# xswang/xflow

Measured on NVIDIA H100. Metric: training examples/sec, higher is better.
Workload: dtype f32

## Files before the change

### xflow_b200/csrc/step_lazy.cu

```cuda
#include <cuda_runtime.h>
#include <stdint.h>
#include <stdlib.h>

#include "kernels.h"
#include "table.cuh"

#define XF_NO_SLOT 0xFFFFFFFFu
#define XF_LAZY_CACHED 2

template <bool ADMIT, bool STAMP>
__device__ __forceinline__ bool xf_lazy_look(const XfTableView& t, uint64_t key, uint64_t& s, uint32_t& i, uint64_t& q0,
                                             uint64_t& q1, uint64_t& q2, uint64_t& q3, uint32_t& slot, bool& created,
                                             const XfAdmitView& adm, bool& rejected, const XfStampView& sv) {
  if (q0 == key) { slot = (uint32_t)s; return true; }
  if (q0 == XF_EMPTY_KEY) {
    if (ADMIT && !xf_admit(adm, key)) {
      rejected = adm.mode != XF_ADM_NEVER;
      return true;
    }
    const unsigned long long old =
        atomicCAS(reinterpret_cast<unsigned long long*>(xf_row(t, s)), (unsigned long long)XF_EMPTY_KEY, (unsigned long long)key);
    if (old == XF_EMPTY_KEY) {
      if (STAMP) sv.stamp[s] = sv.now;
      created = true;
      q0 = key; q1 = q2 = q3 = 0ull;
      slot = (uint32_t)s;
      return true;
    }
    if (old == key) {
      q0 = key;
      slot = (uint32_t)s;
      return true;
    }
  }
  if (++i == XF_MAX_PROBE) { *t.error = 1; return true; }
  s = xf_probe_slot(t, key, i);
  return false;
}

template <bool ADMIT, bool STAMP, bool WEIGHT>
__global__ void __launch_bounds__(256, 2)
xf_k_step_lr_lazy(XfTableView t, const uint32_t* __restrict__ row_ptr, const uint64_t* __restrict__ keys,
                  const uint8_t* __restrict__ labels, int B, int mode, uint32_t seq, uint64_t* rows_by_seq, int fix_shift,
                  float* __restrict__ loss_out, float* __restrict__ pctr_out, float* __restrict__ abs_loss_sum,
                  unsigned long long* __restrict__ unique_total, XfAdmitView adm, XfStampView sv, XfWeightView wv) {
  __shared__ float s_abs[8];
  __shared__ unsigned int s_open;
  if (WEIGHT) fix_shift = xf_fix_shift(*wv.W);
  __shared__ uint64_t s_q2[2 * XF_LAZY_CACHED][256], s_q3[2 * XF_LAZY_CACHED][256], s_q2n[2 * XF_LAZY_CACHED][256];
  if (threadIdx.x == 0) s_open = 0;
  if (blockIdx.x == 0 && threadIdx.x == 0 && mode == 0)
    rows_by_seq[seq] = (uint64_t)(uint32_t)B | ((uint64_t)fix_shift << 32);
  __syncthreads();
  float abs_acc = 0.f;
  unsigned int open_acc = 0;
  const int lane = threadIdx.x & 31;
  const int warps_per_block = blockDim.x >> 5;
  const int gwarp = blockIdx.x * warps_per_block + (threadIdx.x >> 5);
  const int nwarps = gridDim.x * warps_per_block;

  for (int row = gwarp; row < B; row += nwarps) {
    if (WEIGHT && __ldg(wv.e + row) == 0.f) {
      if (lane == 0 && loss_out) loss_out[row] = 0.f;
      continue;
    }
    const uint32_t beg = __ldg(row_ptr + row);
    const uint32_t end = __ldg(row_ptr + row + 1);
    const int chunks = (int)((end - beg + 63u) >> 6);
    const uint8_t label = mode == 0 ? labels[row] : 0;
    uint64_t k1_0 = 0ull, k1_1 = 0ull;
    if (beg + 64u + (uint32_t)lane < end) k1_0 = __ldcs(keys + beg + 64u + lane);
    if (beg + 96u + (uint32_t)lane < end) k1_1 = __ldcs(keys + beg + 96u + lane);
    float wsum = 0.f;
    uint32_t lead_s[2 * XF_LAZY_CACHED];
    uint32_t cnt_c[XF_LAZY_CACHED];
#pragma unroll
    for (int c = 0; c < XF_LAZY_CACHED; ++c) {
      lead_s[2 * c] = lead_s[2 * c + 1] = XF_NO_SLOT;
      cnt_c[c] = 0;
    }

    for (int ch = 0; ch < chunks; ++ch) {
      const uint32_t j0 = beg + (uint32_t)ch * 64u + (uint32_t)lane;
      const uint32_t j1 = j0 + 32u;
      const bool v0 = j0 < end, v1 = j1 < end;
      uint64_t k0 = k1_0, k1 = k1_1;
      if (ch != 1) {
        k0 = v0 ? __ldcs(keys + j0) : 0ull;
        k1 = v1 ? __ldcs(keys + j1) : 0ull;
      }
      uint64_t p0 = xf_home_slot(t, k0), p1 = xf_home_slot(t, k1);
      uint64_t a0, a1, a2, a3, b0, b1, b2, b3;
      xf_ld32_pair(v0 ? xf_row(t, p0) : nullptr, a0, a1, a2, a3);
      xf_ld32_pair(v1 ? xf_row(t, p1) : nullptr, b0, b1, b2, b3);
      uint32_t s0 = XF_NO_SLOT, s1 = XF_NO_SLOT, i0 = 0, i1 = 0;
      bool u0 = v0, u1 = v1, r0 = false, r1 = false;
      for (;;) {
        bool c0 = false, c1 = false;
        if (u0) u0 = !xf_lazy_look<ADMIT, STAMP>(t, k0, p0, i0, a0, a1, a2, a3, s0, c0, adm, r0, sv);
        if (u1) u1 = !xf_lazy_look<ADMIT, STAMP>(t, k1, p1, i1, b0, b1, b2, b3, s1, c1, adm, r1, sv);
        const unsigned created = __popc(__ballot_sync(0xffffffffu, c0)) + __popc(__ballot_sync(0xffffffffu, c1));
        if (created && lane == 0) {
          atomicAdd(t.size, (unsigned long long)created);
          if (ADMIT) atomicAdd(adm.admitted, (unsigned long long)created);
        }
        if (!__any_sync(0xffffffffu, u0 || u1)) break;
        uint64_t x0, x1, x2, x3;
        xf_ld32_pair(u0 ? xf_row(t, p0) : nullptr, x0, x1, x2, x3);
        if (u0) { a0 = x0; a1 = x1; a2 = x2; a3 = x3; }
        xf_ld32_pair(u1 ? xf_row(t, p1) : nullptr, x0, x1, x2, x3);
        if (u1) { b0 = x0; b1 = x1; b2 = x2; b3 = x3; }
      }
      if (ADMIT) xf_admit_append(adm, r0, k0, r1, k1);
      uint64_t a2n = a2, b2n = b2;
      float w0 = 0.f, w1 = 0.f;
      if (s0 != XF_NO_SLOT) w0 = xf_lazy_fold(t, a1, a2, a3, mode == 1 ? 0xFFFFFFFFu : seq, a2n);
      if (s1 != XF_NO_SLOT) w1 = xf_lazy_fold(t, b1, b2, b3, mode == 1 ? 0xFFFFFFFFu : seq, b2n);
      wsum += w0;
      wsum += w1;
      if (mode == 1) continue;
      const unsigned grp0 = __match_any_sync(0xffffffffu, (s0 != XF_NO_SLOT) ? s0 : (0xFFFFFF00u | (uint32_t)lane));
      const unsigned grp1 = __match_any_sync(0xffffffffu, (s1 != XF_NO_SLOT) ? s1 : (0xFFFFFF00u | (uint32_t)lane));
      const bool L0 = s0 != XF_NO_SLOT && lane == __ffs(grp0) - 1, L1 = s1 != XF_NO_SLOT && lane == __ffs(grp1) - 1;
      if (ch >= XF_LAZY_CACHED) {
        if (L0 && xf_lazy_deposit(t, xf_row(t, s0), a2, a3, a2n, seq, 0ll)) {
          ++open_acc;
          if (STAMP) sv.stamp[s0] = sv.now;
        }
        if (L1 && xf_lazy_deposit(t, xf_row(t, s1), b2, b3, b2n, seq, 0ll)) {
          ++open_acc;
          if (STAMP) sv.stamp[s1] = sv.now;
        }
      }
#pragma unroll
      for (int c = 0; c < XF_LAZY_CACHED; ++c)
        if (ch == c) {
          lead_s[2 * c] = L0 ? s0 : XF_NO_SLOT;
          lead_s[2 * c + 1] = L1 ? s1 : XF_NO_SLOT;
          cnt_c[c] = (L0 ? (uint32_t)__popc(grp0) : 0u) | ((L1 ? (uint32_t)__popc(grp1) : 0u) << 8);
        }
      if (ch < XF_LAZY_CACHED) {
        if (L0) { s_q2[2 * ch][threadIdx.x] = a2; s_q3[2 * ch][threadIdx.x] = a3; s_q2n[2 * ch][threadIdx.x] = a2n; }
        if (L1) { s_q2[2 * ch + 1][threadIdx.x] = b2; s_q3[2 * ch + 1][threadIdx.x] = b3; s_q2n[2 * ch + 1][threadIdx.x] = b2n; }
      }
    }

    const float wx = xf_warp_sum(wsum);
    const float pctr = xf_sigmoid(wx);
    if (mode == 1) {
      if (lane == 0 && pctr_out) pctr_out[row] = pctr;
      continue;
    }
    float loss = __fsub_rn(pctr, (float)label);
    if (lane == 0 && loss_out) loss_out[row] = loss;
    if (WEIGHT) loss = __fmul_rn(__ldg(wv.e + row), loss);
    abs_acc += fabsf(loss);
    const long long lf = xf_fix_of(loss, fix_shift);
    uint64_t o2[2 * XF_LAZY_CACHED], o3[2 * XF_LAZY_CACHED];
    bool issued[2 * XF_LAZY_CACHED];
#pragma unroll
    for (int g = 0; g < 2 * XF_LAZY_CACHED; ++g) {
      const int x = threadIdx.x;
      issued[g] = lead_s[g] != XF_NO_SLOT &&
                  xf_lazy_deposit_issue(xf_row(t, lead_s[g]), s_q2[g][x], s_q3[g][x], s_q2n[g][x], seq,
                                        lf * (long long)((cnt_c[g >> 1] >> (8 * (g & 1))) & 0xFFu), o2[g], o3[g]);
    }
#pragma unroll
    for (int g = 0; g < 2 * XF_LAZY_CACHED; ++g) {
      const int x = threadIdx.x;
      bool stale = false;
      if (issued[g] && xf_lazy_deposit_resolve(xf_row(t, lead_s[g]), true, s_q2[g][x], s_q3[g][x], o2[g], o3[g], seq,
                                               lf * (long long)((cnt_c[g >> 1] >> (8 * (g & 1))) & 0xFFu), &stale)) {
        ++open_acc;
        if (STAMP) sv.stamp[lead_s[g]] = sv.now;
      }
      if (stale) *t.error = 2;
    }
    for (int ch = XF_LAZY_CACHED; ch < chunks; ++ch) {
      const uint32_t j0 = beg + (uint32_t)ch * 64u + (uint32_t)lane;
      const uint32_t j1 = j0 + 32u;
      XfHead h;
      if (j0 < end) { const int64_t r = xf_probe<false>(t, __ldg(keys + j0), &h); if (r >= 0) xf_lazy_add(xf_row(t, (uint64_t)r), lf); }
      if (j1 < end) { const int64_t r = xf_probe<false>(t, __ldg(keys + j1), &h); if (r >= 0) xf_lazy_add(xf_row(t, (uint64_t)r), lf); }
    }
  }
  if (mode == 0) {
    if (lane == 0) s_abs[threadIdx.x >> 5] = abs_acc;
    if (open_acc) atomicAdd(&s_open, open_acc);
    __syncthreads();
    if (threadIdx.x == 0) {
      if (abs_loss_sum != nullptr) {
        float tot = 0.f;
        for (int w = 0; w < (int)(blockDim.x >> 5); ++w) tot += s_abs[w];
        atomicAdd(abs_loss_sum, tot);
      }
      if (unique_total != nullptr && s_open) atomicAdd(unique_total, (unsigned long long)s_open);
    }
  }
}

template <bool A, bool S, bool W>
static int xf_lazy_ctas_per_sm() {
  static const int n = [] {
    int v = 0;
    if (cudaOccupancyMaxActiveBlocksPerMultiprocessor(&v, xf_k_step_lr_lazy<A, S, W>, 256, 0) != cudaSuccess || v < 1) {
      cudaGetLastError();
      v = 1;
    }
    return v;
  }();
  return n;
}

void xf_launch_step_lr_lazy(const XfTableView& t, const uint32_t* row_ptr, const uint64_t* keys,
                            const uint8_t* labels, int B, uint64_t nnz, int mode, uint32_t seq, uint64_t* rows_by_seq,
                            float* loss_out, float* pctr_out, float* abs_loss_sum, unsigned long long* unique_total,
                            const XfAdmitView* adm, const XfStampView& sv, const XfWeightView& wv, cudaStream_t st) {
  if (B <= 0) return;
  const int fs = xf_fix_shift(nnz);
  const XfAdmitView a = adm ? *adm : XfAdmitView{};
#define XF_LAZY_ARGS t, row_ptr, keys, labels, B, mode, seq, rows_by_seq, fs, loss_out, pctr_out, abs_loss_sum, unique_total, a, sv, wv
#define XF_LAZY_LAUNCH(A, S, W)                                                                                      \
  xf_k_step_lr_lazy<A, S, W><<<xf_grid_for((uint64_t)B * 32, 256, xf_lazy_ctas_per_sm<A, S, W>()), 256, 0, st>>>( \
      XF_LAZY_ARGS)
#define XF_LAZY_LAUNCH_W(A, S)            \
  do {                                    \
    if (wv.e) XF_LAZY_LAUNCH(A, S, true); \
    else XF_LAZY_LAUNCH(A, S, false);     \
  } while (0)
  const bool stamp = sv.stamp != nullptr;
  if (adm && stamp) XF_LAZY_LAUNCH_W(true, true);
  else if (adm) XF_LAZY_LAUNCH_W(true, false);
  else if (stamp) XF_LAZY_LAUNCH_W(false, true);
  else XF_LAZY_LAUNCH_W(false, false);
#undef XF_LAZY_LAUNCH_W
#undef XF_LAZY_LAUNCH
#undef XF_LAZY_ARGS
}
```

### xflow_b200/csrc/table.cuh

```cuda
#pragma once
#include <cuda_runtime.h>
#include <stdint.h>

#define XF_EMPTY_KEY 0xFFFFFFFFFFFFFFFFull
#define XF_FLAG_V_READY 1u
#define XF_NEG_ZERO_BITS 0x80000000u
#define XF_NEG_ZERO_BITS64 0x8000000000000000ull
#define XF_MAX_PROBE 8192

enum { XF_OPT_FTRL = 0, XF_OPT_SGD = 1 };
enum { XF_INIT_DEFAULT = 0, XF_INIT_COUNTER = 1, XF_INIT_ZERO = 3 };

struct XfTableView {
  uint8_t* base;
  uint64_t mask;
  uint32_t log2cap;
  uint32_t bshift;
  uint32_t stride;
  int K;
  int opt;
  int v_init;
  float v_const;
  uint64_t seed;
  float alpha, beta, lambda1, lambda2, learning_rate;
  unsigned long long* size;
  int* error;
  int lazy;
  const uint64_t* rows_by_seq;
  int canon;
};
#define XF_ADM_POISSON 1
#define XF_ADM_BLOOM 2
#define XF_ADM_NEVER 3
#define XF_ADM_MAX_HASHES 8
struct XfAdmitView {
  int mode;
  uint32_t p24;
  uint64_t batch_mix;
  uint32_t threshold, log2_cells, hashes;
  uint64_t seed;
  const uint8_t* cells;
  unsigned long long* rej_n;
  uint64_t* rej_keys;
  unsigned long long* admitted;
};
struct XfKeep {
  uint32_t cutoff;
  int bounded;
  uint32_t s_star;
  uint64_t k_star;
};
struct XfStampView {
  uint32_t* stamp;
  uint32_t now;
};
struct XfWeightView {
  const float* e;
  const unsigned long long* W;
};
__host__ __device__ __forceinline__ bool xf_keeps(const XfKeep& k, uint32_t stamp, uint64_t key) {
  return stamp >= k.cutoff && (!k.bounded || stamp > k.s_star || (stamp == k.s_star && key <= k.k_star));
}
#define XF_TAG_LOCKED 0xFFFFFFFFu
#define XF_FIX_MAX_SHIFT 27
#define XF_TAG_MASK 0xFFFFull

__host__ __device__ inline int xf_fix_shift(uint64_t nnz) {
  int bits = 0;
  while (bits < 64 && (nnz >> bits) != 0ull) ++bits;
  const int s = 47 - bits;
  return s > XF_FIX_MAX_SHIFT ? XF_FIX_MAX_SHIFT : (s < 0 ? 0 : s);
}

__host__ __device__ inline uint32_t xf_acc_off(int K) { return (32u + 4u * (uint32_t)K + 15u) & ~15u; }
__host__ __device__ inline uint32_t xf_ca_off(int K, int opt) {
  return xf_acc_off(K) + 16u + ((opt == XF_OPT_FTRL) ? 8u * (uint32_t)K : 0u);
}
__host__ __device__ inline uint32_t xf_row_stride(int K, int opt, int canon = 0) {
  if (K <= 0) return 32u;
  uint32_t bytes = xf_ca_off(K, opt) + (canon ? 4u * (uint32_t)K : 0u);
  return (bytes + 31u) & ~31u;
}

#ifdef __CUDACC__

__device__ __forceinline__ uint64_t xf_probe_slot(const XfTableView& t, uint64_t key, uint32_t i) {
  const uint64_t m = key * 0x9E3779B97F4A7C15ull;
  const uint32_t bs = t.bshift;
  const uint64_t hb = m >> (64 - (t.log2cap - bs));
  const uint32_t b1 = (1u << bs) - 1u;
  const uint32_t j0 = (uint32_t)(m >> 9) & b1;
  const uint32_t k = i >> bs;
  const uint32_t j = (k == 0) ? ((j0 + i) & b1) : (i & b1);
  return (((hb + k) << bs) | j) & t.mask;
}
__device__ __forceinline__ uint64_t xf_home_slot(const XfTableView& t, uint64_t key) { return xf_probe_slot(t, key, 0); }

__host__ __device__ __forceinline__ uint64_t xf_splitmix64(uint64_t x) {
  x += 0x9E3779B97F4A7C15ull;
  x = (x ^ (x >> 30)) * 0xBF58476D1CE4E5B9ull;
  x = (x ^ (x >> 27)) * 0x94D049BB133111EBull;
  return x ^ (x >> 31);
}
__host__ __device__ __forceinline__ uint64_t xf_admit_cell(uint64_t key, uint64_t seed, uint32_t j, uint32_t log2_cells) {
  return xf_splitmix64(key ^ xf_splitmix64(seed + (uint64_t)(j + 1) * 0x9E3779B97F4A7C15ull)) >> (64 - log2_cells);
}
__device__ __forceinline__ bool xf_admit(const XfAdmitView& a, uint64_t key) {
  if (a.mode == XF_ADM_POISSON) return (uint32_t)(xf_splitmix64(key ^ a.batch_mix) >> 40) < a.p24;
  if (a.mode != XF_ADM_BLOOM) return false;
  uint32_t m = 255u;
  for (uint32_t j = 0; j < a.hashes; ++j) m = min(m, (uint32_t)__ldcg(a.cells + xf_admit_cell(key, a.seed, j, a.log2_cells)));
  return m >= a.threshold;
}
__device__ __forceinline__ void xf_admit_append(const XfAdmitView& a, bool r0, uint64_t k0, bool r1, uint64_t k1) {
  const unsigned m0 = __ballot_sync(0xffffffffu, r0), m1 = __ballot_sync(0xffffffffu, r1);
  if ((m0 | m1) == 0u) return;
  const unsigned lane = threadIdx.x & 31u;
  unsigned long long base = 0ull;
  if (lane == 0u) base = atomicAdd(a.rej_n, (unsigned long long)(__popc(m0) + __popc(m1)));
  base = __shfl_sync(0xffffffffu, base, 0);
  if (a.rej_keys) {
    const unsigned lt = (1u << lane) - 1u;
    if (r0) a.rej_keys[base + __popc(m0 & lt)] = k0;
    if (r1) a.rej_keys[base + __popc(m0) + __popc(m1 & lt)] = k1;
  }
}

__device__ __forceinline__ float xf_counter_normal(uint64_t key, uint32_t k, uint64_t seed) {
  uint64_t base = xf_splitmix64(key ^ xf_splitmix64(seed + 0x632BE59BD9B4E019ull * (uint64_t)(k + 1)));
  uint32_t sum = 0;
#pragma unroll
  for (int r = 0; r < 3; ++r) {
    uint64_t x = xf_splitmix64(base + (uint64_t)r);
    sum += (uint32_t)(x & 0xFFFF) + (uint32_t)((x >> 16) & 0xFFFF) + (uint32_t)((x >> 32) & 0xFFFF) +
           (uint32_t)((x >> 48) & 0xFFFF);
  }
  float u = __fmul_rn((float)((int32_t)sum - 6 * 65535), 1.0f / 65536.0f);
  return __fmul_rn(u, 1e-2f);
}
__device__ __forceinline__ float xf_v_init(const XfTableView& t, uint64_t key, uint32_t k) {
  if (t.v_init == XF_INIT_COUNTER) return xf_counter_normal(key, k, t.seed);
  if (t.v_init == XF_INIT_ZERO) return 0.0f;
  return t.v_const;
}

__device__ __forceinline__ uint8_t* xf_row(const XfTableView& t, uint64_t slot) {
  return t.base + slot * (uint64_t)t.stride;
}
__device__ __forceinline__ double* xf_row_g(uint8_t* row) { return reinterpret_cast<double*>(row + 8); }
#define XF_OFF_STATE 16
#define XF_OFF_FLAGS 28
__device__ __forceinline__ float* xf_row_v(uint8_t* row) { return reinterpret_cast<float*>(row + 32); }
__device__ __forceinline__ double* xf_row_acc(uint8_t* row, int K) { return reinterpret_cast<double*>(row + xf_acc_off(K)); }
__device__ __forceinline__ float* xf_row_nv(uint8_t* row, int K) { return reinterpret_cast<float*>(row + xf_acc_off(K) + 16); }
__device__ __forceinline__ float* xf_row_zv(uint8_t* row, int K) { return xf_row_nv(row, K) + K; }
__device__ __forceinline__ float* xf_row_ca(const XfTableView& t, uint8_t* row) { return reinterpret_cast<float*>(row + xf_ca_off(t.K, t.opt)); }

struct XfHead {
  uint64_t key;
  uint32_t flags;
  float w, n, z;
  double g;
};

__device__ __forceinline__ void xf_ld32_cg(const void* p, uint64_t& q0, uint64_t& q1, uint64_t& q2, uint64_t& q3) {
  asm volatile("ld.global.cg.v2.u64 {%0,%1}, [%4];\n\tld.global.cg.v2.u64 {%2,%3}, [%4+16];"
               : "=l"(q0), "=l"(q1), "=l"(q2), "=l"(q3) : "l"(p));
}
__device__ __forceinline__ void xf_ld32_ca(const void* p, uint64_t& q0, uint64_t& q1, uint64_t& q2, uint64_t& q3) {
  asm volatile("ld.global.ca.v2.u64 {%0,%1}, [%4];\n\tld.global.ca.v2.u64 {%2,%3}, [%4+16];"
               : "=l"(q0), "=l"(q1), "=l"(q2), "=l"(q3) : "l"(p));
}
__device__ __forceinline__ void xf_ld32_pair(const uint8_t* mine, uint64_t& q0, uint64_t& q1, uint64_t& q2, uint64_t& q3) {
  const uint32_t odd = threadIdx.x & 1u;
  const uint8_t* other = (const uint8_t*)__shfl_xor_sync(0xffffffffu, (unsigned long long)mine, 1);
  const uint8_t* r0 = odd ? other : mine;
  const uint8_t* r1 = odd ? mine : other;
  uint64_t x0 = 0, x1 = 0, y0 = 0, y1 = 0;
  asm volatile("{\n .reg .pred p0, p1;\n setp.ne.u64 p0, %4, 0;\n setp.ne.u64 p1, %5, 0;\n"
               " @p0 ld.global.cg.v2.u64 {%0,%1}, [%6];\n @p1 ld.global.cg.v2.u64 {%2,%3}, [%7];\n}"
               : "+l"(x0), "+l"(x1), "+l"(y0), "+l"(y1)
               : "l"(r0), "l"(r1), "l"(r0 + 16 * odd), "l"(r1 + 16 * odd));
  const uint64_t m0 = odd ? y0 : x0, m1 = odd ? y1 : x1;
  const uint64_t t0 = __shfl_xor_sync(0xffffffffu, odd ? x0 : y0, 1);
  const uint64_t t1 = __shfl_xor_sync(0xffffffffu, odd ? x1 : y1, 1);
  q0 = odd ? t0 : m0; q1 = odd ? t1 : m1;
  q2 = odd ? m0 : t0; q3 = odd ? m1 : t1;
}
__device__ __forceinline__ void xf_st32(void* p, uint64_t q0, uint64_t q1, uint64_t q2, uint64_t q3) {
  asm volatile("st.global.v2.u64 [%0], {%1,%2};\n\tst.global.v2.u64 [%0+16], {%3,%4};" ::"l"(p), "l"(q0), "l"(q1),
               "l"(q2), "l"(q3)
               : "memory");
}

__device__ __forceinline__ XfHead xf_load_head(const uint8_t* row) {
  uint64_t q0, q1, q2, q3;
  xf_ld32_cg(row, q0, q1, q2, q3);
  XfHead h;
  h.key = q0;
  h.g = __longlong_as_double((long long)q1);
  h.w = __uint_as_float((uint32_t)q2);
  h.n = __uint_as_float((uint32_t)(q2 >> 32));
  h.z = __uint_as_float((uint32_t)q3);
  h.flags = (uint32_t)(q3 >> 32);
  return h;
}

__device__ __forceinline__ XfHead xf_load_head_l1(const uint8_t* row) {
  uint64_t q0, q1, q2, q3;
  xf_ld32_ca(row, q0, q1, q2, q3);
  XfHead h;
  h.key = q0;
  h.g = __longlong_as_double((long long)q1);
  h.w = __uint_as_float((uint32_t)q2);
  h.n = __uint_as_float((uint32_t)(q2 >> 32));
  h.z = __uint_as_float((uint32_t)q3);
  h.flags = (uint32_t)(q3 >> 32);
  return h;
}

__device__ __forceinline__ void xf_ld8_l1(const float* p, float (&o)[8]) {
  uint64_t q0, q1, q2, q3;
  xf_ld32_ca(p, q0, q1, q2, q3);
  o[0] = __uint_as_float((uint32_t)q0); o[1] = __uint_as_float((uint32_t)(q0 >> 32));
  o[2] = __uint_as_float((uint32_t)q1); o[3] = __uint_as_float((uint32_t)(q1 >> 32));
  o[4] = __uint_as_float((uint32_t)q2); o[5] = __uint_as_float((uint32_t)(q2 >> 32));
  o[6] = __uint_as_float((uint32_t)q3); o[7] = __uint_as_float((uint32_t)(q3 >> 32));
}

template <int VEC>
__device__ __forceinline__ void xf_ldv_step(const float* p, float (&o)[VEC]) {
  if (VEC == 4) { float4 t = __ldca(reinterpret_cast<const float4*>(p)); o[0] = t.x; o[1 % VEC] = t.y; o[2 % VEC] = t.z; o[3 % VEC] = t.w; }
  else if (VEC == 2) { float2 t = __ldca(reinterpret_cast<const float2*>(p)); o[0] = t.x; o[1 % VEC] = t.y; }
  else { o[0] = __ldca(p); }
}
template <int VEC>
__device__ __forceinline__ void xf_fm_token(const XfTableView& t, uint32_t slot, uint32_t flags, uint64_t key,
                                            float& st, float& qt) {
  const int K = t.K;
  st = 0.f;
  qt = 0.f;
  if ((flags & XF_FLAG_V_READY) && (K & 7) == 0) {
    const float* vp = reinterpret_cast<const float*>(xf_row(t, slot) + 32);
    for (int k = 0; k < K; k += 8) {
      float v[8];
      xf_ld8_l1(vp + k, v);
#pragma unroll
      for (int e = 0; e < 8; ++e) { st += v[e]; qt = __fadd_rn(qt, __fmul_rn(v[e], v[e])); }
    }
  } else if (flags & XF_FLAG_V_READY) {
    const float* vp = reinterpret_cast<const float*>(xf_row(t, slot) + 32);
    for (int k = 0; k < K; k += VEC) {
      float v[VEC];
      xf_ldv_step<VEC>(vp + k, v);
#pragma unroll
      for (int e = 0; e < VEC; ++e) { st += v[e]; qt = __fadd_rn(qt, __fmul_rn(v[e], v[e])); }
    }
  } else {
    for (int k = 0; k < K; ++k) {
      const float v = xf_v_init(t, key, (uint32_t)k);
      st += v;
      qt = __fadd_rn(qt, __fmul_rn(v, v));
    }
  }
}

__device__ __forceinline__ void xf_store_head(uint8_t* row, const XfHead& h) {
  const uint64_t q1 = (uint64_t)__double_as_longlong(h.g);
  const uint64_t q2 = (uint64_t)__float_as_uint(h.w) | ((uint64_t)__float_as_uint(h.n) << 32);
  const uint64_t q3 = (uint64_t)__float_as_uint(h.z) | ((uint64_t)h.flags << 32);
  xf_st32(row, h.key, q1, q2, q3);
}

template <bool INSERT, bool ADMIT = false, bool STAMP = false>
__device__ __forceinline__ int64_t xf_probe_from(const XfTableView& t, uint64_t key, uint64_t s, XfHead& h,
                                                 const XfAdmitView* adm = nullptr, bool* rejected = nullptr,
                                                 const XfStampView* sv = nullptr) {
  for (int probes = 0; probes < XF_MAX_PROBE; ++probes) {
    if (h.key == key) return (int64_t)s;
    if (h.key == XF_EMPTY_KEY) {
      if (!INSERT) return -1;
      if (ADMIT && !xf_admit(*adm, key)) {
        *rejected = adm->mode != XF_ADM_NEVER;
        return -1;
      }
      unsigned long long old =
          atomicCAS(reinterpret_cast<unsigned long long*>(xf_row(t, s)), (unsigned long long)XF_EMPTY_KEY,
                    (unsigned long long)key);
      if (old == XF_EMPTY_KEY) {
        unsigned m = __activemask();
        int leader = __ffs(m) - 1;
        if ((int)(threadIdx.x & 31) == leader) {
          atomicAdd(t.size, (unsigned long long)__popc(m));
          if (ADMIT) atomicAdd(adm->admitted, (unsigned long long)__popc(m));
        }
        if (STAMP && sv->stamp != nullptr) sv->stamp[s] = sv->now;
        h.key = key; h.flags = 0; h.w = 0.f; h.n = 0.f; h.z = 0.f;
        h.g = t.lazy ? 0.0 : -0.0;
        return (int64_t)s;
      }
      if (old == key) {
        h.key = key;
        return (int64_t)s;
      }
    }
    s = xf_probe_slot(t, key, (uint32_t)probes + 1u);
    h = xf_load_head(xf_row(t, s));
  }
  *t.error = 1;
  return -1;
}

template <bool INSERT, bool STAMP = false>
__device__ __forceinline__ int64_t xf_probe(const XfTableView& t, uint64_t key, XfHead* head,
                                            const XfStampView* sv = nullptr) {
  const uint64_t s = xf_home_slot(t, key);
  XfHead h = xf_load_head(xf_row(t, s));
  const int64_t r = xf_probe_from<INSERT, false, STAMP>(t, key, s, h, nullptr, nullptr, sv);
  *head = h;
  return r;
}


__device__ __forceinline__ float xf_sigmoid(float x) {
  if (x < -30.f) return (float)1e-6;
  if (x > 30.f) return 1.0f;
  const double ex = exp((double)x * 0.9999999998311266);
  return (float)(ex / (1.0 + ex));
}

__device__ __forceinline__ void xf_ftrl_coord(const XfTableView& t, float g, float& w, float& n, float& z) {
  float old_n = n;
  float nn = __fadd_rn(old_n, __fmul_rn(g, g));
  float sig = __fdiv_rn(__fsub_rn(__fsqrt_rn(nn), __fsqrt_rn(old_n)), t.alpha);
  z = __fadd_rn(z, __fsub_rn(g, __fmul_rn(sig, w)));
  n = nn;
  if (fabsf(z) <= t.lambda1) {
    w = 0.0f;
  } else {
    float tmpr = 0.0f;
    if (z > 0.0f) tmpr = __fsub_rn(z, t.lambda1);
    if (z < 0.0f) tmpr = __fadd_rn(z, t.lambda1);
    float tmpl = -__fadd_rn(__fdiv_rn(__fadd_rn(t.beta, __fsqrt_rn(n)), t.alpha), t.lambda2);
    w = __fdiv_rn(tmpr, tmpl);
  }
}

__device__ __forceinline__ void xf_sgd_coord(const XfTableView& t, float g, float& w) {
  w = __fsub_rn(w, __fmul_rn(t.learning_rate, g));
}

__device__ __forceinline__ void xf_opt_coord(const XfTableView& t, float g, float& w, float& n, float& z) {
  if (t.opt == XF_OPT_FTRL) xf_ftrl_coord(t, g, w, n, z);
  else xf_sgd_coord(t, g, w);
}

__device__ __forceinline__ float xf_div_rows_plain(float g, double rows) { return (float)((double)g / rows); }
__device__ __forceinline__ float xf_div_rows(float g, double rows) {
  const long long b = __double_as_longlong(rows);
  if ((b & 0x000FFFFFFFFFFFFFll) == 0ll && b > 0ll) {
    const double inv = __longlong_as_double((2046ll << 52) - b);
    return (float)((double)g * inv);
  }
  return (float)((double)g / rows);
}

__device__ __forceinline__ float xf_ftrl_w(const XfTableView& t, float z, float n) {
  if (fabsf(z) <= t.lambda1) return 0.0f;
  float tmpr = 0.0f;
  if (z > 0.0f) tmpr = __fsub_rn(z, t.lambda1);
  if (z < 0.0f) tmpr = __fadd_rn(z, t.lambda1);
  const float tmpl = -__fadd_rn(__fdiv_rn(__fadd_rn(t.beta, __fsqrt_rn(n)), t.alpha), t.lambda2);
  return __fdiv_rn(tmpr, tmpl);
}
__device__ __forceinline__ double xf_pow2(int e) { return __longlong_as_double((long long)(1023 + e) << 52); }
__device__ __forceinline__ long long xf_fix_of(float residual, int shift) {
  return __double2ll_rn((double)residual * xf_pow2(shift));
}

__device__ __forceinline__ uint64_t xf_raw_q2(const XfHead& h) {
  return (uint64_t)__float_as_uint(h.w) | ((uint64_t)__float_as_uint(h.n) << 32);
}
__device__ __forceinline__ uint64_t xf_raw_q3(const XfHead& h) {
  return (uint64_t)__float_as_uint(h.z) | ((uint64_t)h.flags << 32);
}
__device__ __forceinline__ uint64_t xf_raw_q1(const XfHead& h) { return (uint64_t)__double_as_longlong(h.g); }
__device__ __forceinline__ uint32_t xf_lazy_check(uint64_t q2) {
  const uint32_t c = (uint32_t)q2 ^ (uint32_t)(q2 >> 32) ^ 0xA5A5A5A5u;
  return c ? c : 1u;
}
__device__ __forceinline__ float xf_lazy_fold(const XfTableView& t, uint64_t q1, uint64_t q2, uint64_t q3, uint32_t seq,
                                              uint64_t& q2_new) {
  const uint32_t tag = (uint32_t)(q3 & XF_TAG_MASK);
  const bool pending = tag != 0u && tag != seq;
  float g = 0.f;
  if (pending) {
    const long long gfix = (long long)q3 >> 16;
    const uint64_t rs = __ldg(t.rows_by_seq + tag);
    g = xf_div_rows_plain((float)((double)gfix * xf_pow2(-(int)(rs >> 32))), (double)(uint32_t)rs);
  }
  const float a = __uint_as_float((uint32_t)q2), b = __uint_as_float((uint32_t)(q2 >> 32));
  if (t.opt == XF_OPT_FTRL) {
    float n = a, z = b;
    float w = ((uint32_t)(q1 >> 32) == xf_lazy_check(q2)) ? __uint_as_float((uint32_t)q1) : xf_ftrl_w(t, z, n);
    if (pending) xf_ftrl_coord(t, g, w, n, z);
    q2_new = (uint64_t)__float_as_uint(n) | ((uint64_t)__float_as_uint(z) << 32);
    return w;
  }
  float w = a;
  if (pending) xf_sgd_coord(t, g, w);
  q2_new = (uint64_t)__float_as_uint(w);
  return w;
}
__device__ __forceinline__ void xf_apply_pending(const XfTableView& t, XfHead& h) {
  if (!t.lazy) return;
  uint64_t q2n;
  const float w = xf_lazy_fold(t, xf_raw_q1(h), xf_raw_q2(h), xf_raw_q3(h), 0xFFFFFFFFu, q2n);
  h.w = w;
  if (t.opt == XF_OPT_FTRL) {
    h.n = __uint_as_float((uint32_t)q2n);
    h.z = __uint_as_float((uint32_t)(q2n >> 32));
  } else {
    h.n = 0.f;
    h.z = 0.f;
  }
  h.flags = 0u;
  h.g = 0.0;
}
__device__ __forceinline__ bool xf_lazy_has_pending(const XfHead& raw) { return (xf_raw_q3(raw) & XF_TAG_MASK) != 0ull; }
__device__ __forceinline__ void xf_lazy_store(const XfTableView& t, uint8_t* rowp, const XfHead& h, bool keep_w = false) {
  const bool ftrl = t.opt == XF_OPT_FTRL;
  const uint64_t q2 = ftrl ? ((uint64_t)__float_as_uint(h.n) | ((uint64_t)__float_as_uint(h.z) << 32))
                           : (uint64_t)__float_as_uint(h.w);
  uint64_t q1 = 0ull;
  if (keep_w && ftrl && __float_as_uint(h.w) != __float_as_uint(xf_ftrl_w(t, h.z, h.n)))
    q1 = (uint64_t)__float_as_uint(h.w) | ((uint64_t)xf_lazy_check(q2) << 32);
  xf_st32(rowp, h.key, q1, q2, 0ull);
}
__device__ __forceinline__ void xf_store_head_t(const XfTableView& t, uint8_t* rowp, const XfHead& h) {
  if (t.lazy) xf_lazy_store(t, rowp, h);
  else xf_store_head(rowp, h);
}

__device__ __forceinline__ bool xf_cas128(uint8_t* addr, uint64_t e0, uint64_t e1, uint64_t d0, uint64_t d1, uint64_t& o0,
                                          uint64_t& o1) {
  asm volatile(
      "{\n .reg .b128 cmp, swp, old;\n mov.b128 cmp, {%2, %3};\n mov.b128 swp, {%4, %5};\n"
      " atom.global.cas.b128 old, [%6], cmp, swp;\n mov.b128 {%0, %1}, old;\n}"
      : "=l"(o0), "=l"(o1)
      : "l"(e0), "l"(e1), "l"(d0), "l"(d1), "l"(addr)
      : "memory");
  return o0 == e0 && o1 == e1;
}
__device__ __forceinline__ void xf_lazy_add(uint8_t* rowp, long long fix) {
  atomicAdd(reinterpret_cast<unsigned long long*>(rowp + 24), (unsigned long long)fix << 16);
}
__device__ __forceinline__ bool xf_lazy_deposit_issue(uint8_t* rowp, uint64_t q2, uint64_t q3, uint64_t q2_new, uint32_t seq,
                                                      long long fix, uint64_t& o2, uint64_t& o3) {
  if ((uint32_t)(q3 & XF_TAG_MASK) == seq) {
    xf_lazy_add(rowp, fix);
    o2 = q2; o3 = q3;
    return false;
  }
  xf_cas128(rowp + XF_OFF_STATE, q2, q3, q2_new, ((unsigned long long)fix << 16) | (uint64_t)seq, o2, o3);
  return true;
}
__device__ __forceinline__ bool xf_lazy_deposit_resolve(uint8_t* rowp, bool issued, uint64_t q2, uint64_t q3, uint64_t o2,
                                                        uint64_t o3, uint32_t seq, long long fix, bool* stale) {
  *stale = false;
  if (!issued) return false;
  if (o2 == q2 && o3 == q3) return true;
  if ((uint32_t)(o3 & XF_TAG_MASK) == seq) {
    xf_lazy_add(rowp, fix);
    return false;
  }
  *stale = true;
  return false;
}
__device__ __forceinline__ bool xf_lazy_deposit(const XfTableView& t, uint8_t* rowp, uint64_t q2, uint64_t q3, uint64_t q2_new,
                                                uint32_t seq, long long fix, bool* stale = nullptr) {
  if (stale) *stale = false;
  if ((uint32_t)(q3 & XF_TAG_MASK) == seq) {
    xf_lazy_add(rowp, fix);
    return false;
  }
  uint64_t o2, o3;
  if (xf_cas128(rowp + XF_OFF_STATE, q2, q3, q2_new, ((unsigned long long)fix << 16) | (uint64_t)seq, o2, o3)) return true;
  if ((uint32_t)(o3 & XF_TAG_MASK) == seq) {
    xf_lazy_add(rowp, fix);
    return false;
  }
  if (stale) *stale = true;
  else *t.error = 2;
  return false;
}

__device__ __forceinline__ float xf_warp_sum(float v) {
#pragma unroll
  for (int o = 16; o > 0; o >>= 1) v += __shfl_xor_sync(0xffffffffu, v, o);
  return v;
}

#endif
```

Measured before the change: 87.26 million.

## Process each row with a multi-warp thread group using named barriers

Measured after the change: 92.78 million, median of 6. 6.3% higher.

```diff
diff --git a/xflow_b200/csrc/step_lazy.cu b/xflow_b200/csrc/step_lazy.cu
--- a/xflow_b200/csrc/step_lazy.cu
+++ b/xflow_b200/csrc/step_lazy.cu
@@ -6,7 +6,6 @@
 #include "table.cuh"
 
 #define XF_NO_SLOT 0xFFFFFFFFu
-#define XF_LAZY_CACHED 2
 
 template <bool ADMIT, bool STAMP>
 __device__ __forceinline__ bool xf_lazy_look(const XfTableView& t, uint64_t key, uint64_t& s, uint32_t& i, uint64_t& q0,
@@ -38,150 +37,128 @@
   return false;
 }
 
+__device__ __forceinline__ void xf_group_sync(int grp, int n) {
+  switch (grp) {
+    case 0: asm volatile("bar.sync 1, %0;" ::"r"(n) : "memory"); break;
+    case 1: asm volatile("bar.sync 2, %0;" ::"r"(n) : "memory"); break;
+    case 2: asm volatile("bar.sync 3, %0;" ::"r"(n) : "memory"); break;
+    default: asm volatile("bar.sync 4, %0;" ::"r"(n) : "memory"); break;
+  }
+}
+
 template <bool ADMIT, bool STAMP, bool WEIGHT>
-__global__ void __launch_bounds__(256, 2)
+__global__ void __launch_bounds__(256, 4)
 xf_k_step_lr_lazy(XfTableView t, const uint32_t* __restrict__ row_ptr, const uint64_t* __restrict__ keys,
                   const uint8_t* __restrict__ labels, int B, int mode, uint32_t seq, uint64_t* rows_by_seq, int fix_shift,
-                  float* __restrict__ loss_out, float* __restrict__ pctr_out, float* __restrict__ abs_loss_sum,
+                  int gshift, float* __restrict__ loss_out, float* __restrict__ pctr_out, float* __restrict__ abs_loss_sum,
                   unsigned long long* __restrict__ unique_total, XfAdmitView adm, XfStampView sv, XfWeightView wv) {
+  __shared__ float s_w[256];
+  __shared__ long long s_lf[4];
   __shared__ float s_abs[8];
   __shared__ unsigned int s_open;
   if (WEIGHT) fix_shift = xf_fix_shift(*wv.W);
-  __shared__ uint64_t s_q2[2 * XF_LAZY_CACHED][256], s_q3[2 * XF_LAZY_CACHED][256], s_q2n[2 * XF_LAZY_CACHED][256];
   if (threadIdx.x == 0) s_open = 0;
   if (blockIdx.x == 0 && threadIdx.x == 0 && mode == 0)
     rows_by_seq[seq] = (uint64_t)(uint32_t)B | ((uint64_t)fix_shift << 32);
   __syncthreads();
   float abs_acc = 0.f;
   unsigned int open_acc = 0;
+  const int G = 1 << gshift;
   const int lane = threadIdx.x & 31;
-  const int warps_per_block = blockDim.x >> 5;
-  const int gwarp = blockIdx.x * warps_per_block + (threadIdx.x >> 5);
-  const int nwarps = gridDim.x * warps_per_block;
-
-  for (int row = gwarp; row < B; row += nwarps) {
+  const int x = threadIdx.x & (G - 1);
+  const int grp = threadIdx.x >> gshift;
+  const int gbase = grp << gshift;
+  const bool summer = x < 32;
+  const int groups_per_block = blockDim.x >> gshift;
+
+  for (int row = blockIdx.x * groups_per_block + grp; row < B; row += gridDim.x * groups_per_block) {
     if (WEIGHT && __ldg(wv.e + row) == 0.f) {
-      if (lane == 0 && loss_out) loss_out[row] = 0.f;
+      if (x == 0 && loss_out) loss_out[row] = 0.f;
       continue;
     }
     const uint32_t beg = __ldg(row_ptr + row);
     const uint32_t end = __ldg(row_ptr + row + 1);
-    const int chunks = (int)((end - beg + 63u) >> 6);
-    const uint8_t label = mode == 0 ? labels[row] : 0;
-    uint64_t k1_0 = 0ull, k1_1 = 0ull;
-    if (beg + 64u + (uint32_t)lane < end) k1_0 = __ldcs(keys + beg + 64u + lane);
-    if (beg + 96u + (uint32_t)lane < end) k1_1 = __ldcs(keys + beg + 96u + lane);
+    const int rounds = (int)((end - beg + (uint32_t)G - 1u) >> gshift);
+    const uint8_t label = (mode == 0 && summer) ? labels[row] : 0;
     float wsum = 0.f;
-    uint32_t lead_s[2 * XF_LAZY_CACHED];
-    uint32_t cnt_c[XF_LAZY_CACHED];
-#pragma unroll
-    for (int c = 0; c < XF_LAZY_CACHED; ++c) {
-      lead_s[2 * c] = lead_s[2 * c + 1] = XF_NO_SLOT;
-      cnt_c[c] = 0;
-    }
-
-    for (int ch = 0; ch < chunks; ++ch) {
-      const uint32_t j0 = beg + (uint32_t)ch * 64u + (uint32_t)lane;
-      const uint32_t j1 = j0 + 32u;
-      const bool v0 = j0 < end, v1 = j1 < end;
-      uint64_t k0 = k1_0, k1 = k1_1;
-      if (ch != 1) {
-        k0 = v0 ? __ldcs(keys + j0) : 0ull;
-        k1 = v1 ? __ldcs(keys + j1) : 0ull;
-      }
-      uint64_t p0 = xf_home_slot(t, k0), p1 = xf_home_slot(t, k1);
-      uint64_t a0, a1, a2, a3, b0, b1, b2, b3;
-      xf_ld32_pair(v0 ? xf_row(t, p0) : nullptr, a0, a1, a2, a3);
-      xf_ld32_pair(v1 ? xf_row(t, p1) : nullptr, b0, b1, b2, b3);
-      uint32_t s0 = XF_NO_SLOT, s1 = XF_NO_SLOT, i0 = 0, i1 = 0;
-      bool u0 = v0, u1 = v1, r0 = false, r1 = false;
+    uint32_t lead_s = XF_NO_SLOT, cnt = 0;
+    uint64_t lq2 = 0ull, lq3 = 0ull, lq2n = 0ull;
+
+    for (int rd = 0; rd < rounds; ++rd) {
+      const uint32_t j = beg + ((uint32_t)rd << gshift) + (uint32_t)x;
+      const bool v = j < end;
+      const uint64_t k = v ? __ldcs(keys + j) : 0ull;
+      uint64_t p = xf_home_slot(t, k);
+      uint64_t a0, a1, a2, a3;
+      xf_ld32_pair(v ? xf_row(t, p) : nullptr, a0, a1, a2, a3);
+      uint32_t s = XF_NO_SLOT, i = 0;
+      bool u = v, r = false;
       for (;;) {
-        bool c0 = false, c1 = false;
-        if (u0) u0 = !xf_lazy_look<ADMIT, STAMP>(t, k0, p0, i0, a0, a1, a2, a3, s0, c0, adm, r0, sv);
-        if (u1) u1 = !xf_lazy_look<ADMIT, STAMP>(t, k1, p1, i1, b0, b1, b2, b3, s1, c1, adm, r1, sv);
-        const unsigned created = __popc(__ballot_sync(0xffffffffu, c0)) + __popc(__ballot_sync(0xffffffffu, c1));
+        bool c = false;
+        if (u) u = !xf_lazy_look<ADMIT, STAMP>(t, k, p, i, a0, a1, a2, a3, s, c, adm, r, sv);
+        const unsigned created = __popc(__ballot_sync(0xffffffffu, c));
         if (created && lane == 0) {
           atomicAdd(t.size, (unsigned long long)created);
           if (ADMIT) atomicAdd(adm.admitted, (unsigned long long)created);
         }
-        if (!__any_sync(0xffffffffu, u0 || u1)) break;
+        if (!__any_sync(0xffffffffu, u)) break;
         uint64_t x0, x1, x2, x3;
-        xf_ld32_pair(u0 ? xf_row(t, p0) : nullptr, x0, x1, x2, x3);
-        if (u0) { a0 = x0; a1 = x1; a2 = x2; a3 = x3; }
-        xf_ld32_pair(u1 ? xf_row(t, p1) : nullptr, x0, x1, x2, x3);
-        if (u1) { b0 = x0; b1 = x1; b2 = x2; b3 = x3; }
-      }
-      if (ADMIT) xf_admit_append(adm, r0, k0, r1, k1);
-      uint64_t a2n = a2, b2n = b2;
-      float w0 = 0.f, w1 = 0.f;
-      if (s0 != XF_NO_SLOT) w0 = xf_lazy_fold(t, a1, a2, a3, mode == 1 ? 0xFFFFFFFFu : seq, a2n);
-      if (s1 != XF_NO_SLOT) w1 = xf_lazy_fold(t, b1, b2, b3, mode == 1 ? 0xFFFFFFFFu : seq, b2n);
-      wsum += w0;
-      wsum += w1;
-      if (mode == 1) continue;
-      const unsigned grp0 = __match_any_sync(0xffffffffu, (s0 != XF_NO_SLOT) ? s0 : (0xFFFFFF00u | (uint32_t)lane));
-      const unsigned grp1 = __match_any_sync(0xffffffffu, (s1 != XF_NO_SLOT) ? s1 : (0xFFFFFF00u | (uint32_t)lane));
-      const bool L0 = s0 != XF_NO_SLOT && lane == __ffs(grp0) - 1, L1 = s1 != XF_NO_SLOT && lane == __ffs(grp1) - 1;
-      if (ch >= XF_LAZY_CACHED) {
-        if (L0 && xf_lazy_deposit(t, xf_row(t, s0), a2, a3, a2n, seq, 0ll)) {
+        xf_ld32_pair(u ? xf_row(t, p) : nullptr, x0, x1, x2, x3);
+        if (u) { a0 = x0; a1 = x1; a2 = x2; a3 = x3; }
+      }
+      if (ADMIT) xf_admit_append(adm, r, k);
+      uint64_t a2n = a2;
+      float w = 0.f;
+      if (s != XF_NO_SLOT) w = xf_lazy_fold(t, a1, a2, a3, mode == 1 ? 0xFFFFFFFFu : seq, a2n);
+      s_w[threadIdx.x] = w;
+      if (mode == 0) {
+        const unsigned gm = __match_any_sync(0xffffffffu, (s != XF_NO_SLOT) ? s : (0xFFFFFF00u | (uint32_t)lane));
+        const bool L = s != XF_NO_SLOT && lane == __ffs(gm) - 1;
+        if (rd == 0) {
+          if (L) { lead_s = s; cnt = (uint32_t)__popc(gm); lq2 = a2; lq3 = a3; lq2n = a2n; }
+        } else if (L && xf_lazy_deposit(t, xf_row(t, s), a2, a3, a2n, seq, 0ll)) {
           ++open_acc;
-          if (STAMP) sv.stamp[s0] = sv.now;
+          if (STAMP) sv.stamp[s] = sv.now;
         }
-        if (L1 && xf_lazy_deposit(t, xf_row(t, s1), b2, b3, b2n, seq, 0ll)) {
-          ++open_acc;
-          if (STAMP) sv.stamp[s1] = sv.now;
-        }
-      }
-#pragma unroll
-      for (int c = 0; c < XF_LAZY_CACHED; ++c)
-        if (ch == c) {
-          lead_s[2 * c] = L0 ? s0 : XF_NO_SLOT;
-          lead_s[2 * c + 1] = L1 ? s1 : XF_NO_SLOT;
-          cnt_c[c] = (L0 ? (uint32_t)__popc(grp0) : 0u) | ((L1 ? (uint32_t)__popc(grp1) : 0u) << 8);
-        }
-      if (ch < XF_LAZY_CACHED) {
-        if (L0) { s_q2[2 * ch][threadIdx.x] = a2; s_q3[2 * ch][threadIdx.x] = a3; s_q2n[2 * ch][threadIdx.x] = a2n; }
-        if (L1) { s_q2[2 * ch + 1][threadIdx.x] = b2; s_q3[2 * ch + 1][threadIdx.x] = b3; s_q2n[2 * ch + 1][threadIdx.x] = b2n; }
-      }
-    }
-
-    const float wx = xf_warp_sum(wsum);
-    const float pctr = xf_sigmoid(wx);
-    if (mode == 1) {
-      if (lane == 0 && pctr_out) pctr_out[row] = pctr;
-      continue;
-    }
-    float loss = __fsub_rn(pctr, (float)label);
-    if (lane == 0 && loss_out) loss_out[row] = loss;
-    if (WEIGHT) loss = __fmul_rn(__ldg(wv.e + row), loss);
-    abs_acc += fabsf(loss);
-    const long long lf = xf_fix_of(loss, fix_shift);
-    uint64_t o2[2 * XF_LAZY_CACHED], o3[2 * XF_LAZY_CACHED];
-    bool issued[2 * XF_LAZY_CACHED];
-#pragma unroll
-    for (int g = 0; g < 2 * XF_LAZY_CACHED; ++g) {
-      const int x = threadIdx.x;
-      issued[g] = lead_s[g] != XF_NO_SLOT &&
-                  xf_lazy_deposit_issue(xf_row(t, lead_s[g]), s_q2[g][x], s_q3[g][x], s_q2n[g][x], seq,
-                                        lf * (long long)((cnt_c[g >> 1] >> (8 * (g & 1))) & 0xFFu), o2[g], o3[g]);
-    }
-#pragma unroll
-    for (int g = 0; g < 2 * XF_LAZY_CACHED; ++g) {
-      const int x = threadIdx.x;
+      }
+      xf_group_sync(grp, G);
+      if (summer)
+        for (int o = 0; o < G; o += 32) wsum += s_w[gbase + o + lane];
+      if (rd + 1 < rounds) xf_group_sync(grp, G);
+    }
+
+    if (summer) {
+      const float wx = xf_warp_sum(wsum);
+      const float pctr = xf_sigmoid(wx);
+      if (mode == 1) {
+        if (lane == 0 && pctr_out) pctr_out[row] = pctr;
+      } else {
+        float loss = __fsub_rn(pctr, (float)label);
+        if (lane == 0 && loss_out) loss_out[row] = loss;
+        if (WEIGHT) loss = __fmul_rn(__ldg(wv.e + row), loss);
+        abs_acc += fabsf(loss);
+        if (lane == 0 && rounds > 0) s_lf[grp] = xf_fix_of(loss, fix_shift);
+      }
+    }
+    xf_group_sync(grp, G);
+    if (mode == 1 || rounds == 0) continue;
+    const long long lf = s_lf[grp];
+    if (lead_s != XF_NO_SLOT) {
+      uint8_t* rowp = xf_row(t, lead_s);
+      const long long fix = lf * (long long)cnt;
+      uint64_t o2, o3;
       bool stale = false;
-      if (issued[g] && xf_lazy_deposit_resolve(xf_row(t, lead_s[g]), true, s_q2[g][x], s_q3[g][x], o2[g], o3[g], seq,
-                                               lf * (long long)((cnt_c[g >> 1] >> (8 * (g & 1))) & 0xFFu), &stale)) {
+      const bool issued = xf_lazy_deposit_issue(rowp, lq2, lq3, lq2n, seq, fix, o2, o3);
+      if (issued && xf_lazy_deposit_resolve(rowp, true, lq2, lq3, o2, o3, seq, fix, &stale)) {
         ++open_acc;
-        if (STAMP) sv.stamp[lead_s[g]] = sv.now;
+        if (STAMP) sv.stamp[lead_s] = sv.now;
       }
       if (stale) *t.error = 2;
     }
-    for (int ch = XF_LAZY_CACHED; ch < chunks; ++ch) {
-      const uint32_t j0 = beg + (uint32_t)ch * 64u + (uint32_t)lane;
-      const uint32_t j1 = j0 + 32u;
+    for (int rd = 1; rd < rounds; ++rd) {
+      const uint32_t j = beg + ((uint32_t)rd << gshift) + (uint32_t)x;
       XfHead h;
-      if (j0 < end) { const int64_t r = xf_probe<false>(t, __ldg(keys + j0), &h); if (r >= 0) xf_lazy_add(xf_row(t, (uint64_t)r), lf); }
-      if (j1 < end) { const int64_t r = xf_probe<false>(t, __ldg(keys + j1), &h); if (r >= 0) xf_lazy_add(xf_row(t, (uint64_t)r), lf); }
+      if (j < end) { const int64_t r = xf_probe<false>(t, __ldg(keys + j), &h); if (r >= 0) xf_lazy_add(xf_row(t, (uint64_t)r), lf); }
     }
   }
   if (mode == 0) {
@@ -219,9 +196,10 @@
   if (B <= 0) return;
   const int fs = xf_fix_shift(nnz);
   const XfAdmitView a = adm ? *adm : XfAdmitView{};
-#define XF_LAZY_ARGS t, row_ptr, keys, labels, B, mode, seq, rows_by_seq, fs, loss_out, pctr_out, abs_loss_sum, unique_total, a, sv, wv
-#define XF_LAZY_LAUNCH(A, S, W)                                                                                      \
-  xf_k_step_lr_lazy<A, S, W><<<xf_grid_for((uint64_t)B * 32, 256, xf_lazy_ctas_per_sm<A, S, W>()), 256, 0, st>>>( \
+  const int gshift = nnz <= 64ull * (uint64_t)B ? 6 : 7;
+#define XF_LAZY_ARGS t, row_ptr, keys, labels, B, mode, seq, rows_by_seq, fs, gshift, loss_out, pctr_out, abs_loss_sum, unique_total, a, sv, wv
+#define XF_LAZY_LAUNCH(A, S, W)                                                                                        \
+  xf_k_step_lr_lazy<A, S, W><<<xf_grid_for((uint64_t)B << gshift, 256, xf_lazy_ctas_per_sm<A, S, W>()), 256, 0, st>>>( \
       XF_LAZY_ARGS)
 #define XF_LAZY_LAUNCH_W(A, S)            \
   do {                                    \
diff --git a/xflow_b200/csrc/table.cuh b/xflow_b200/csrc/table.cuh
--- a/xflow_b200/csrc/table.cuh
+++ b/xflow_b200/csrc/table.cuh
@@ -125,6 +125,15 @@
     if (r1) a.rej_keys[base + __popc(m0) + __popc(m1 & lt)] = k1;
   }
 }
+__device__ __forceinline__ void xf_admit_append(const XfAdmitView& a, bool r, uint64_t k) {
+  const unsigned m = __ballot_sync(0xffffffffu, r);
+  if (m == 0u) return;
+  const unsigned lane = threadIdx.x & 31u;
+  unsigned long long base = 0ull;
+  if (lane == 0u) base = atomicAdd(a.rej_n, (unsigned long long)__popc(m));
+  base = __shfl_sync(0xffffffffu, base, 0);
+  if (a.rej_keys && r) a.rej_keys[base + __popc(m & ((1u << lane) - 1u))] = k;
+}
 
 __device__ __forceinline__ float xf_counter_normal(uint64_t key, uint32_t k, uint64_t seed) {
   uint64_t base = xf_splitmix64(key ^ xf_splitmix64(seed + 0x632BE59BD9B4E019ull * (uint64_t)(k + 1)));
```
